# OpenwaterHealth/OpenLIFU-python

Hardware: AMD Instinct MI355X
Metric: Mvoxel-elements/s pressure-field accumulate (higher is better)
Workload: dtype f32-acc/f16x2+e4m3-corr

## Files before the change

### openlifu-python_amd/csrc/k_coset2.hip

```cpp
#include <algorithm>
#include <cstdlib>
#include "k_types.hip.h"
#include "olx_ctx.h"
#include "olx_launch.h"

namespace olx {

constexpr int CP_TW = 14;
constexpr int CP_TROWS = 26, CP_ROW0 = 15;
constexpr int CP_PSZ = 364;
constexpr int CP_UW = 12;
constexpr int CP_MT = 5;

#ifdef OLX_EXP_CUTRACE
static __device__ unsigned long long g_cutrace[16384][8][5];
#define OLX_CUTRACE(k, v) do { if (lane == 0 && blockIdx.y == 0 && blockIdx.x < 16384) g_cutrace[blockIdx.x][wave][k] = (v); } while (0)
#else
#define OLX_CUTRACE(k, v)
#endif

template <int MX, int MY, bool CLAMP, bool FP8, bool DIR = false, bool BOTH = true >
__global__ __launch_bounds__(COS_NW * 64, 4) void field_cosetp_k(
    const uint4* __restrict__ bfrag, float* __restrict__ pmag, float* __restrict__ inten,
    const int* __restrict__ targets ,
    const CosetBlock* __restrict__ blocks , const CosetParams P) {
    constexpr int NT = 2, THREADS = COS_NW * 64, PAIR = 2;
    constexpr int TROWS = CP_TROWS, ROW0 = CP_ROW0, PSZ = CP_PSZ, MT = CP_MT;
    static_assert((PSZ / 2) % 2 == 0 && ((PSZ / 2) % 32 == 22 || (PSZ / 2) % 32 == 30), "16 planes on 16 distinct even 8-byte slots");
    constexpr int RPR = 64 / CP_UW, NROUND = (TROWS + RPR - 1) / RPR;
    constexpr int B_KS_U4 = 128;
    constexpr int B_BYTES = PAIR * 4 * NT * B_KS_U4 * 16;
    constexpr int T_WORDS = COS_ZB * PSZ;
    __shared__ __attribute__((aligned(16))) unsigned char smem[B_BYTES + T_WORDS * 4 + T_WORDS * 4 + 64];
    auto s_B = [&](int rec, int nt, int part) -> const uint4* { return reinterpret_cast<const uint4*>(smem) + ((size_t)(rec * NT + nt) * B_KS_U4 + part * 64); };
    unsigned* const s_hi = reinterpret_cast<unsigned*>(smem + B_BYTES);
    unsigned* const s_lo = s_hi + T_WORDS;
    const int tile = blockIdx.y;
    const int tid = threadIdx.x, lane = tid & 63, wave = __builtin_amdgcn_readfirstlane(tid >> 6);
    const int g = lane >> 4, p16 = lane & 15;
    OLX_CUTRACE(2, __builtin_readcyclecounter());
    OLX_CUTRACE(0, (unsigned long long)__builtin_amdgcn_s_getreg((31 << 11) | 4));
    OLX_CUTRACE(1, (unsigned long long)__builtin_amdgcn_s_getreg((31 << 11) | 20));
    const int item = blockIdx.x;
    {
    const CosetBlock BK = blocks[item];
    const int npos = BK.npos, KY = BK.KY, ky_magic = BK.ky_magic;
    if (npos <= 0) return;
    const int ibase = BK.ibase, jbase = BK.jbase;
    const int k0 = BK.k0;
    const int ntile = __builtin_amdgcn_readfirstlane((npos - wave + COS_NW - 1) / COS_NW);
    const int lane_off = p16 * PSZ - g * CP_TW;
    int toff[MT];
#pragma unroll
    for (int t = 0; t < MT; ++t) {
        const int pos = min(wave + COS_NW * t, npos - 1);
        const int kx = (pos * ky_magic) >> 16, ky = pos - kx * KY;
        toff[t] = (ky + ROW0) * CP_TW + (CP_UW - 8 - 2 * kx);
    }
    floatx4_t acc[MT][NT];
#pragma unroll
    for (int t = 0; t < MT; ++t)
#pragma unroll
        for (int nt = 0; nt < NT; ++nt) acc[t][nt] = floatx4_t{0.f, 0.f, 0.f, 0.f};
    const int nsbp = P.nsbp;
    const int n_sb = P.nsa * nsbp;
    constexpr int CHUNK_U4 = PAIR * 4 * NT * B_KS_U4, PRE = CHUNK_U4 / THREADS;
    static_assert(CHUNK_U4 % THREADS == 0, "chunk must split evenly over the block");
    uint4 pre[PRE];
    const uint4* const bsrc = bfrag + (size_t)tile * n_sb * (4 * NT * B_KS_U4);
#pragma unroll
    for (int q = 0; q < PRE; ++q) {
        const int idx = tid + q * THREADS;
        pre[q] = idx < n_sb * 4 * NT * B_KS_U4 ? bsrc[idx] : make_uint4(0, 0, 0, 0);
    }
    OLX_STAMP(0);
    for (int sb0 = 0; sb0 < n_sb; sb0 += PAIR) {
        const int sa = sb0 / nsbp, sbb0 = sb0 - sa * nsbp;
        if (sb0 > 0) __syncthreads();
        if (sb0 == 0) OLX_STAMP(1);
        if (sb0 == 2) OLX_STAMP(7);
        if constexpr (FP8) __builtin_amdgcn_s_setprio(1);
        if (k0 + wave * COS_P < P.nz) {
            int lane_o = lane;
            asm volatile("" : "+v"(lane_o));
            const int wl = lane_o / CP_UW, ui = lane_o - CP_UW * wl;
            const bool gen_lane = wl < RPR;
            const int Ulane = ibase + P.x_begin + P.ux0 + P.mx * (ui - 7);
            const int Wlane = jbase + P.uy0 + P.my * (wl - ROW0);
            const int tw_off = (wave * COS_P) * PSZ + wl * CP_TW + (CP_UW - 1 - ui);
            float dz2[COS_P];
#pragma unroll
            for (int z = 0; z < COS_P; ++z) {
                const float dz = (float)(k0 + wave * COS_P + z) * P.hz - P.flat_ez;
                dz2[z] = dz * dz;
            }
            const float U = (float)(Ulane - 8 * P.mx * sa);
            const float dx = fmaf(U, P.hx_hi, fmaf(U, P.hx_lo, P.fx0));
            const float dx2 = dx * dx;
            const int Wsb = Wlane - 8 * P.my * sbb0;
            auto entry = [&](const float r2, const float dz2v, const float dy, const int o, const bool ok) __attribute__((always_inline)) {
                float d2 = r2 + dz2v;
                if (CLAMP) d2 = fmaxf(d2, P.dmin2);
                const float ri = __builtin_amdgcn_rsqf(d2);
                const float ph = d2 * ri;
                float rs = ri * P.g_scale;
                if constexpr (DIR) rs *= table_mod(dx, dy, ph, ri, P.dir_wx, P.dir_wy, P.absorb_l2);
                float gr = rs * __builtin_amdgcn_cosf(ph), gi = rs * __builtin_amdgcn_sinf(ph);
                asm volatile("" : "+v"(gr), "+v"(gi));
                half2_t hi;
                if constexpr (FP8) hi = __builtin_convertvector(float2_t{gr, gi}, half2_t);
                else hi = __builtin_bit_cast(half2_t, __builtin_amdgcn_cvt_pkrtz(gr, gi));
                float lr, li;
                const unsigned hw = __builtin_bit_cast(unsigned, hi);
                asm("v_fma_mix_f32 %0, %1, -1.0, %2 op_sel:[0,0,0] op_sel_hi:[1,0,0]" : "=v"(lr) : "v"(hw), "v"(gr));
                asm("v_fma_mix_f32 %0, %1, -1.0, %2 op_sel:[1,0,0] op_sel_hi:[1,0,0]" : "=v"(li) : "v"(hw), "v"(gi));
                unsigned lo_word;
                if constexpr (FP8) {
                    short2_t w;
                    w = __builtin_amdgcn_cvt_scalef32_pk_fp8_f32(w, lr, li, 1.0f / COS_F8_LO, false);
                    w = __builtin_amdgcn_cvt_scalef32_pk_fp8_f32(w, gr, gi, 1.0f / COS_F8_HI, true);
                    lo_word = __builtin_bit_cast(unsigned, w);
                } else {
                    lo_word = __builtin_bit_cast(unsigned, __builtin_amdgcn_cvt_pkrtz(lr, li));
                }
                if (ok && OLX_IN(o, T_WORDS, 0)) {
                    s_hi[o] = __builtin_bit_cast(unsigned, hi);
                    s_lo[o] = lo_word;
                }
            };
            static_assert((TROWS - 1) % RPR == 0 && COS_P <= RPR, "the last table row is shared by the planes of a wave");
#pragma unroll 2
            for (int r = 0; r < NROUND - 1; ++r) {
                const float W = (float)(Wsb + RPR * P.my * r);
                const float dy = fmaf(W, P.hy_hi, fmaf(W, P.hy_lo, P.fy0));
                const float r2 = fmaf(dy, dy, dx2);
#pragma unroll
                for (int z = 0; z < COS_P; ++z) entry(r2, dz2[z], dy, z * PSZ + tw_off + RPR * r * CP_TW, gen_lane);
            }
            if (KY + 14 >= TROWS - 1) {
                const float W = (float)(Wsb - P.my * wl + (TROWS - 1) * P.my);
                const float dy = fmaf(W, P.hy_hi, fmaf(W, P.hy_lo, P.fy0));
                float dzl = dz2[0];
#pragma unroll
                for (int z = 1; z < COS_P; ++z) dzl = wl == z ? dz2[z] : dzl;
                entry(fmaf(dy, dy, dx2), dzl, dy, (wave * COS_P + wl) * PSZ + (TROWS - 1) * CP_TW + (CP_UW - 1 - ui), wl < COS_P);
            }
        }
        if constexpr (FP8) __builtin_amdgcn_s_setprio(0);
#pragma unroll
        for (int q = 0; q < PRE; ++q) reinterpret_cast<uint4*>(smem)[tid + q * THREADS] = pre[q];
        if (sb0 == 0) OLX_STAMP(2);
        __syncthreads();
        if (sb0 == 0) OLX_STAMP(3);
        {
            const int nxt = (sb0 + PAIR) * 4 * NT * B_KS_U4, lim = n_sb * 4 * NT * B_KS_U4;
#pragma unroll
            for (int q = 0; q < PRE; ++q) {
                const int idx = nxt + tid + q * THREADS;
                if (idx < lim) pre[q] = bsrc[idx];
            }
        }
#pragma unroll
        for (int sl = 0; sl < PAIR; ++sl) {
            if (sbb0 + sl >= P.nsb) break;
            if constexpr (FP8) {
#pragma unroll
                for (int kb = 0; kb < 2; ++kb) {
                    Half8Bits bh[2][NT];
                    intx8_t b8[NT];
#pragma unroll
                    for (int nt = 0; nt < NT; ++nt) {
#pragma unroll
                        for (int ka = 0; ka < 2; ++ka) {
                            bh[ka][nt].u = s_B(sl * 4 + 2 * kb + ka, nt, 0)[lane];
                            const uint4 q = s_B(sl * 4 + 2 * kb + ka, nt, 1)[lane];
                            b8[nt][4 * ka + 0] = (int)q.x; b8[nt][4 * ka + 1] = (int)q.y; b8[nt][4 * ka + 2] = (int)q.z; b8[nt][4 * ka + 3] = (int)q.w;
                        }
                    }
// ... 44 lines not shown
                        if (t >= ntile) continue;
                        Half8Bits ah, al;
                        int lo_t = lane_off;
                        asm volatile("" : "+v"(lo_t));
                        const int ro = lo_t + toff[t];
                        if (!OLX_IN(ro + kso, T_WORDS - 3, 1)) continue;
                        const unsigned long long* ph2 = reinterpret_cast<const unsigned long long*>(s_hi + ro + kso);
                        const unsigned long long* pl2 = reinterpret_cast<const unsigned long long*>(s_lo + ro + kso);
                        const unsigned long long h0 = __hip_atomic_load(ph2, __ATOMIC_RELAXED, __HIP_MEMORY_SCOPE_WAVEFRONT);
                        const unsigned long long h1 = __hip_atomic_load(ph2 + 1, __ATOMIC_RELAXED, __HIP_MEMORY_SCOPE_WAVEFRONT);
                        const unsigned long long l0 = __hip_atomic_load(pl2, __ATOMIC_RELAXED, __HIP_MEMORY_SCOPE_WAVEFRONT);
                        const unsigned long long l1 = __hip_atomic_load(pl2 + 1, __ATOMIC_RELAXED, __HIP_MEMORY_SCOPE_WAVEFRONT);
                        ah.w[0] = (unsigned)h0; ah.w[1] = (unsigned)(h0 >> 32); ah.w[2] = (unsigned)h1; ah.w[3] = (unsigned)(h1 >> 32);
                        al.w[0] = (unsigned)l0; al.w[1] = (unsigned)(l0 >> 32); al.w[2] = (unsigned)l1; al.w[3] = (unsigned)(l1 >> 32);
#pragma unroll
                        for (int nt = 0; nt < NT; ++nt) acc[t][nt] = __builtin_amdgcn_mfma_f32_16x16x32_f16(ah.h, bh[nt].h, acc[t][nt], 0, 0, 0);
#pragma unroll
                        for (int nt = 0; nt < NT; ++nt) acc[t][nt] = __builtin_amdgcn_mfma_f32_16x16x32_f16(al.h, bh[nt].h, acc[t][nt], 0, 0, 0);
#pragma unroll
                        for (int nt = 0; nt < NT; ++nt) acc[t][nt] = __builtin_amdgcn_mfma_f32_16x16x32_f16(ah.h, bl[nt].h, acc[t][nt], 0, 0, 0);
                    }
                }
            }
        }
        if (sb0 == 0) OLX_STAMP(4);
    }
    OLX_STAMP(5);
    int lane_e = lane;
    asm volatile("" : "+v"(lane_e));
    const int c16 = lane_e >> 2;
    const int kz = k0 + 4 * (lane_e & 3);
    const int src_lane4 = (16 * (lane_e & 3) + (lane_e >> 2)) * 4;
    const float s_p = P.out_scale, s_i = P.out_scale * P.out_scale * P.inten_scale;
    const bool want_p = (P.flags & 1u) != 0, want_i = (P.flags & 2u) != 0;
#pragma unroll
    for (int t = 0; t < MT; ++t) {
        if (t >= ntile) continue;
        float o[NT][4];
#pragma unroll
        for (int r = 0; r < 4; r += 2) {
            const float2_t re = {acc[t][0][r], acc[t][0][r + 1]}, im = {acc[t][1][r], acc[t][1][r + 1]};
            const float2_t m = __builtin_elementwise_fma(re, re, im * im);
            o[0][r] = __builtin_amdgcn_sqrtf(m.x) * s_p;
            o[0][r + 1] = __builtin_amdgcn_sqrtf(m.y) * s_p;
            const float2_t in = m * float2_t{s_i, s_i};
            o[1][r] = in.x;
            o[1][r + 1] = in.y;
        }
#pragma unroll
        for (int nt = 0; nt < NT; ++nt) {
            floatx4_t v;
            v[0] = __builtin_bit_cast(float, __builtin_amdgcn_ds_bpermute(src_lane4, __builtin_bit_cast(int, o[nt][0])));
            v[1] = __builtin_bit_cast(float, __builtin_amdgcn_ds_bpermute(src_lane4, __builtin_bit_cast(int, o[nt][1])));
            v[2] = __builtin_bit_cast(float, __builtin_amdgcn_ds_bpermute(src_lane4, __builtin_bit_cast(int, o[nt][2])));
            v[3] = __builtin_bit_cast(float, __builtin_amdgcn_ds_bpermute(src_lane4, __builtin_bit_cast(int, o[nt][3])));
            acc[t][nt] = v;
        }
    }
    if (kz < P.nz) {
    const int4 tq = *reinterpret_cast<const int4*>(targets + ((size_t)tile * (MFMA_COLS * MFMA_MAX_NT) + c16) * 4);
    const int xm = P.nx - 1, ym = P.ny - 1;
    const int sxz = P.ny * P.nz;
    auto readout = [&](auto full_c) {
        constexpr bool FULL4 = decltype(full_c)::value != 0;
#pragma unroll
        for (int q = 0; q < 4; ++q) {
            const int code = q == 0 ? tq.x : q == 1 ? tq.y : q == 2 ? tq.z : tq.w;
            if (code < 0) continue;
            const unsigned m = (unsigned)code & 3u;
            const bool fx = (MX == 2) && (m & 1u), fy = (MY == 2) && ((MX == 2) ? (m >> 1) : (m & 1u));
            unsigned fxm = fx ? 0xFFFFFFFFu : 0u, fym = fy ? 0xFFFFFFFFu : 0u;
            asm volatile("" : "+v"(fxm), "+v"(fym));
            const long long fb = (long long)(code >> 2) * P.vox + kz;
            float* const base_p = pmag + fb;
            float* const base_i = inten + fb;
#pragma unroll
            for (int t = 0; t < MT; ++t) {
                if (t >= ntile) continue;
                const int pos = wave + COS_NW * t;
                const int kx = (pos * ky_magic) >> 16, ky = pos - kx * KY;
                const int i = ibase + 2 * P.mx * kx, j = jbase + P.my * ky;
                const unsigned o00 = (unsigned)(i * sxz + j * P.nz);
                const unsigned DX = (unsigned)((xm - 2 * i) * sxz), DY = (unsigned)((ym - 2 * j) * P.nz);
                const unsigned off = o00 + (fxm & DX) + (fym & DY);
                if (!OLX_IN(fb + off + (FULL4 ? 3 : 0), (long long)P.n_foci * P.vox, 2)) continue;
                if constexpr (FULL4) {
                    if (BOTH || want_p) *reinterpret_cast<floatx4u_t*>(base_p + off) = floatx4u_t{acc[t][0][0], acc[t][0][1], acc[t][0][2], acc[t][0][3]};
                    if (BOTH || want_i) *reinterpret_cast<floatx4u_t*>(base_i + off) = floatx4u_t{acc[t][1][0], acc[t][1][1], acc[t][1][2], acc[t][1][3]};
                } else {
#pragma unroll
                    for (int e = 0; e < 4; ++e)
                        if (kz + e < P.nz) {
                            if (BOTH || want_p) base_p[off + e] = acc[t][0][e];
                            if (BOTH || want_i) base_i[off + e] = acc[t][1][e];
                        }
                }
            }
        }
    };
    if (k0 + COS_ZB <= P.nz) readout(IntC<1>{}); else readout(IntC<0>{});
    }
    OLX_STAMP(6);
#ifdef OLX_EXP_CUTRACE
    OLX_CUTRACE(3, __builtin_readcyclecounter());
    asm volatile("s_waitcnt vmcnt(0)" ::: "memory");
    OLX_CUTRACE(4, __builtin_readcyclecounter());
#endif
    }
}

}

using namespace olx;
OLX_BOUNDS_READER(cosetp)

#ifdef OLX_EXP_CUTRACE
extern "C" int olx_exp_read_cutrace_cosetp(unsigned long long* out) {
    return (int)hipMemcpyFromSymbol(out, HIP_SYMBOL(olx::g_cutrace), sizeof(unsigned long long) * 16384 * 8 * 5);
}
#endif
#ifdef OLX_EXP_STAMPS
extern "C" int olx_exp_read_stamps_cosetp(unsigned long long* out) {
    return (int)hipMemcpyFromSymbol(out, HIP_SYMBOL(olx::g_stamps), sizeof(unsigned long long) * 4096 * 8);
}
#endif

template <int MX, int MY>
static void launch_cosetp(olx_ctx* c, const LatticePart& q, float* pm) {
    CosetParams Q = c->cp;
#ifdef OLX_DEBUG_BOUNDS
    if (getenv("OLX_DEBUG_BOUNDS_SELFTEST")) Q.n_foci -= 1;
#endif
    float* inten_exp = c->d_inten;
    const bool clamp = c->clamp || c->lat.clamp;
    dim3 grid(q.n_blocks, c->mp.n_tiles), blk(COS_NW * 64);
    const bool both = (Q.flags & 3u) == 3u;
#define OLX_CP(CL, F8, DR) do { if (both) hipLaunchKernelGGL((field_cosetp_k<MX, MY, CL, F8, DR, true>), grid, blk, 0, c->stream, q.bfrag, pm, inten_exp, c->d_targets, q.blocks, Q); \
                                else hipLaunchKernelGGL((field_cosetp_k<MX, MY, CL, F8, DR, false>), grid, blk, 0, c->stream, q.bfrag, pm, inten_exp, c->d_targets, q.blocks, Q); } while (0)
    if (c->dir_lattice) {
        if (clamp) OLX_CP(true, false, true); else OLX_CP(false, false, true);
    } else if (q.fp8) {
        if (clamp) OLX_CP(true, true, false); else OLX_CP(false, true, false);
    } else {
        if (clamp) OLX_CP(true, false, false); else OLX_CP(false, false, false);
    }
#undef OLX_CP
}

void olx_launch_cosetp(olx_ctx* c, const LatticePart& q, float* pm) {
    if (c->mx == 2 && c->my == 2) launch_cosetp<2, 2>(c, q, pm);
    else if (c->mx == 2) launch_cosetp<2, 1>(c, q, pm);
    else if (c->my == 2) launch_cosetp<1, 2>(c, q, pm);
    else launch_cosetp<1, 1>(c, q, pm);
}
```

### openlifu-python_amd/csrc/olx.hip

```cpp
#include "olx_ctx.h"

#include <dlfcn.h>
#include <unistd.h>

#include <algorithm>
#include <climits>
#include <cmath>
#include <cstring>
#include <thread>

#include "k_small.hip.h"
#include "olx_launch.h"
#include "olx_plan.h"
#include "k_toep.hip.h"

OLX_BOUNDS_READER(small)

template <class T> static int upload_if_changed(olx_ctx* c, DevBuf<T>& d, std::vector<T>& held, const std::vector<T>& v) {
    if (d.capacity() < v.size() || !d) held.clear();
    { int rc = d.reserve(c, v.size()); if (rc) return rc; }
    if (held.size() == v.size() && (v.empty() || !memcmp(held.data(), v.data(), sizeof(T) * v.size()))) return OLX_OK;
    HIPCHK(c, hipMemcpyAsync(d, v.data(), sizeof(T) * v.size(), hipMemcpyHostToDevice, c->stream));
    HIPCHK(c, hipStreamSynchronize(c->stream));
    held = v;
// ... 652 lines not shown
            L.ux0 = (int)std::llround(offx / c->grid.spacing[0]); L.uy0 = (int)std::llround(offy / c->grid.spacing[1]);
            L.fx0 = (float)((offx - L.ux0 * c->grid.spacing[0]) * rev); L.fy0 = (float)((offy - L.uy0 * c->grid.spacing[1]) * rev);
            const double hxw = c->grid.spacing[0] * rev, hyw = c->grid.spacing[1] * rev;
            L.hx_hi = (float)hxw; L.hx_lo = (float)(hxw - (double)L.hx_hi);
            L.hy_hi = (float)hyw; L.hy_lo = (float)(hyw - (double)L.hy_hi);
            L.hz = P.hz; L.dmin2 = P.dmin2; L.flat_ez = P.flat_ez;
            L.g_scale = M.g_scale; L.out_scale = M.out_scale; L.inten_scale = P.inten_scale;
            L.vox = P.vox; L.flags = P.flags;
            const long long tiles16 = coset_tiles16(P.nx - L.x_lo, P.ny - L.y_lo, A.mx, A.my, c->nt);
            c->fp8corr = fp8_want && c->use_coset && cos_fp8(c->nt) && !c->modifier();
            if (c->use_coset) {
                CosetParams& Q = c->cp;
                Q.nx = L.nx; Q.ny = L.ny; Q.nz = L.nz; Q.x_lo = L.x_lo; Q.y_lo = L.y_lo; Q.x_begin = L.x_begin; Q.mx = L.mx; Q.my = L.my;
                const int zb = COS_ZB;
                Q.xs = c->use_toep ? 1 : 2;
                olxplan::ToepPlan tp{};
                c->toep_nm = 1;
                int kyw = COS_KYW;
                if (c->use_toep) {
                    int saw_pin = 0, nm_pin = 0;
#ifdef OLX_DEV_PINS
                    if (const char* e = getenv("OLX_EXP_TOEP_SAW")) { const int v = atoi(e); if (v >= 8 && v <= 24) saw_pin = v; }
                    if (const char* e = getenv("OLX_EXP_TOEP_NM")) nm_pin = atoi(e) == 3 ? 3 : 1;
#endif
                    tp = olxplan::toep_plan(A.ax, Q.mx, Q.my, Q.xs, Q.nx - Q.x_lo, Q.ny - Q.y_lo, Q.nz, c->dir_lattice, saw_pin, nm_pin);
                    c->toep_nm = tp.nm; kyw = tp.kyw;
                }
                const int kxw = c->use_toep ? 8 * c->toep_nm : cos_kxw(c->nt);
                olxplan::coset_partition(Q, kxw, zb, kyw);
                Q.nsa = L.nsa; Q.nsb = L.nsb; Q.nsbp = L.nsbp; Q.ux0 = L.ux0; Q.uy0 = L.uy0; Q.fx0 = L.fx0; Q.fy0 = L.fy0;
                Q.hx_hi = L.hx_hi; Q.hx_lo = L.hx_lo; Q.hy_hi = L.hy_hi; Q.hy_lo = L.hy_lo; Q.hz = L.hz;
                Q.dmin2 = L.dmin2; Q.flat_ez = L.flat_ez; Q.g_scale = L.g_scale; Q.out_scale = L.out_scale; Q.inten_scale = L.inten_scale;
                Q.vox = L.vox; Q.flags = L.flags; Q.n_foci = F;
                Q.dir_wx = (c->dir_lattice && c->directivity) ? (float)(0.5 * c->h_size[0] / lambda) : 0.f;
                Q.dir_wy = (c->dir_lattice && c->directivity) ? (float)(0.5 * c->h_size[1] / lambda) : 0.f;
                Q.absorb_l2 = c->dir_lattice ? (float)(c->absorb_np_m * lambda * 1.4426950408889634) : 0.f;
                {
                    const std::vector<int> jobs = olxplan::build_store_jobs(tiles, MFMA_MAX_NT, MFMA_COLS, COS_JOBS, (P.flags & OLX_OUT_PMAG) != 0, (P.flags & OLX_OUT_INTENSITY) != 0);
                    int rc = upload_if_changed(c, c->d_jobs, c->up_jobs, jobs);
                    if (rc) return rc;
                }
                {
                    auto pick_grp = [&](int kblocks) {
                        const unsigned long long nb = (unsigned long long)Q.xs * Q.mx * Q.my * Q.nsx * Q.nsy * kblocks;
                        for (int g2 = std::min(kblocks, 32); g2 >= 2; --g2) if (kblocks % g2 == 0 && nb % (8ull * g2) == 0) return (unsigned)g2;
                        return 1u;
                    };
                    const int kcut = c->fp8corr ? c->fp8_kcut : 0;
                    const int kb_near = kcut / zb, kb_far = Q.kblocks - kb_near;
                    unsigned kgrp = pick_grp(kb_far), kgrp_near = kb_near > 0 ? pick_grp(kb_near) : 0u;
#ifdef OLX_DEV_PINS
                    if (const char* e = getenv("OLX_EXP_KGRP")) { kgrp = (unsigned)std::max(1, atoi(e)); if (kb_near > 0) kgrp_near = kgrp; }
#endif
                    const int rec_key[16] = {Q.nx, Q.ny, Q.nz, Q.x_lo, Q.y_lo, Q.mx, Q.my, Q.nsx, Q.nsy, Q.kblocks, zb, (int)kgrp, c->use_cosetp ? 40 : 0, Q.xs, kcut, (int)kgrp_near};
                    std::vector<CosetBlock> blk;
                    if (!c->up_blocks.empty() && memcmp(c->up_blocks_key, rec_key, sizeof rec_key) == 0) blk = c->up_blocks;
                    else {
                        std::string why;
                        CosetParams Qf = Q; Qf.kblocks = kb_far;
                        if (!olxplan::build_coset_blocks(Qf, zb, kgrp, c->use_cosetp ? 40 : 0, blk, why))
                            return fail(c, OLX_ESTATE, "kernel 2g: %s", why.c_str());
                        for (CosetBlock& b : blk) b.k0 += kcut;
                        if (kb_near > 0) {
                            std::vector<CosetBlock> near;
                            CosetParams Qn = Q; Qn.kblocks = kb_near;
                            if (!olxplan::build_coset_blocks(Qn, zb, kgrp_near, c->use_cosetp ? 40 : 0, near, why))
// ... 18 lines not shown
                    c->toep_ksmask = tp.ks_mask;
                    const int ksteps_total = tp.ksteps_total, e4_units = tp.e4_units;
                    for (int q = 0; q < 4; ++q) c->toep_targets[q] = tiles[0][0].tgt[q];
                    { int rc = c->d_cell.reserve(c, A.cell.size()); if (rc) return rc; }
                    HIPCHK(c, hipMemcpy(c->d_cell, A.cell.data(), sizeof(int) * A.cell.size(), hipMemcpyHostToDevice));
                    c->afrag_half = (size_t)ntiles * c->toep_nsa * 8 * A.nsb * 4 * 64;
                    { int rc = c->d_afrag.reserve(c, 2 * c->afrag_half); if (rc) return rc; }
                    long long n_mfma = 0;
                    const int wx = P.nx - L.x_lo, wy = P.ny - L.y_lo;
                    const double units_e4m3 = c->toep_nm == 2 ? 3.0 : (double)ksteps_total + (double)e4_units;
                    const double per_row = far_frac * units_e4m3 + (1.0 - far_frac) * 3.0 * ksteps_total;
                    for (int rx = 0; rx < Q.xs * A.mx; ++rx)
                        for (int ry = 0; ry < A.my; ++ry) {
                            const int kxa = rx < wx ? (wx - 1 - rx) / (Q.xs * A.mx) + 1 : 0, kya = ry < wy ? (wy - 1 - ry) / A.my + 1 : 0;
                            for (int sx = 0; sx < Q.nsx; ++sx)
                                for (int sy = 0; sy < Q.nsy; ++sy) {
                                    const int KX = (sx + 1) * kxa / Q.nsx - sx * kxa / Q.nsx, KY = (sy + 1) * kya / Q.nsy - sy * kya / Q.nsy;
                                    if (KX > 0 && KY > 0) n_mfma += (long long)((double)KY * per_row * (c->toep_nm > 1 ? 8 * c->toep_nm : 8) * A.nsb * Q.kblocks);
                                }
                        }
                    snprintf(nmbuf, sizeof nmbuf, "field_toep%s_k<mx%d,my%d,flat,%s%s> %d columns for %d foci x %d images in %d tile(s); "
                             "%dx%d lattice, pitch %dx%d voxels, %lld MFMA/launch (%lld dense), %d row tile(s) x %d y positions per block", "", c->mx, c->my, lat_clamp ? "clamp" : "noclamp", f8tag.c_str(),
                             total_cols, F, n_img, ntiles, A.ax, A.ay, A.mx, A.my, n_mfma, n_dense, c->toep_nm, kyw);
                } else {
                long long n_mfma = (long long)((double)tiles16 * ((P.nz + COS_P - 1) / COS_P) * A.nsa * A.nsb * 4 * c->nt * corr_units * ntiles);
                if (c->use_cosetp) {
                    long long npos_all = 0;
                    const int wx = P.nx - L.x_lo, wy = P.ny - L.y_lo;
                    for (int rx = 0; rx < 2 * A.mx; ++rx)
                        for (int ry = 0; ry < A.my; ++ry)
                            npos_all += (long long)(rx < wx ? (wx - 1 - rx) / (2 * A.mx) + 1 : 0) * (ry < wy ? (wy - 1 - ry) / A.my + 1 : 0);
                    n_mfma = (long long)((double)npos_all * Q.kblocks * A.nsa * A.nsb * 4 * c->nt * corr_units * ntiles);
                }
                snprintf(nmbuf, sizeof nmbuf, "field_coset%s_k<nt%d,mx%d,my%d,flat,%s%s%s> %d columns for %d foci x %d images in %d tile(s); "
                         "%dx%d lattice, pitch %dx%d voxels, %lld MFMA/launch (%lld dense)", c->use_cosetp ? "p" : "", c->nt, c->mx, c->my, lat_clamp ? "clamp" : "noclamp",
                         f8tag.c_str(), "", total_cols, F, n_img, ntiles, A.ax, A.ay, A.mx, A.my, n_mfma, n_dense);
                }
            } else {
                const long long n_mfma = (long long)L.tiles_x * L.tiles_y * L.kgroups * A.nsa * A.nsb * 4 * c->lat_mt * c->nt * 3 * ntiles;
                snprintf(nmbuf, sizeof nmbuf, "field_lattice_k<mt%d,nt%d,mx%d,my%d,flat,%s> %d columns for %d foci x %d images in %d tile(s); "
                         "%dx%d lattice, pitch %dx%d voxels, %lld MFMA/launch", c->lat_mt, c->nt, c->mx, c->my, lat_clamp ? "clamp" : "noclamp",
                         total_cols, F, n_img, ntiles, A.ax, A.ay, A.mx, A.my, n_mfma);
            }
        } else {
            snprintf(nmbuf, sizeof nmbuf, "field_mfma_k<mt%d,nt%d,mx%d,my%d,%s,%s> %d columns for %d foci x %d images in %d tile(s)",
                     P.nz >= 48 ? 4 : 1, c->nt, c->mx, c->my, c->flat ? "flat" : "general", c->clamp ? "clamp" : (c->near ? "near" : "noclamp"), total_cols, F,
                     n_img, ntiles);
        }
    } else if (c->mx * c->my * c->nf == 1) {
        if (c->modifier()) snprintf(nmbuf, sizeof nmbuf, "field_accum_dir_k<4,%s> (%s%s%s)", c->clamp ? "clamp" : "noclamp", c->directivity ? "piston directivity" : "",
                                    (c->directivity && c->absorb_np_m > 0) ? ", " : "", c->absorb_np_m > 0 ? "uniform absorption" : "");
        else snprintf(nmbuf, sizeof nmbuf, "field_accum_k<4,%s,%s>", c->flat ? "flat" : "general", c->clamp ? "clamp" : (c->near ? "near" : "noclamp"));
    } else {
        const std::vector<int> perm = olxplan::mirror_perms(n, nm, c->dx == 2, c->dy == 2, c->h_px.data(), c->h_py.data(), nm);
        int rc = upload_if_changed(c, c->d_perm, c->up_perm, perm);
        if (!rc) rc = c->d_tab.reserve(c, (size_t)((F + c->nf - 1) / c->nf) * n * (SH_HEAD + 2 * nm * c->nf));
        if (rc) return rc;
        snprintf(nmbuf, sizeof nmbuf, "field_shared_k<4,mx%d,my%d,dx%d,dy%d,nf%d,%s,%s>", c->mx, c->my, c->dx, c->dy, c->nf,
                 c->flat ? "flat" : "general", c->clamp ? "clamp" : (c->near ? "near" : "noclamp"));
    }
    if (c->modifier() && c->use_mfma && !(c->use_lattice && c->use_coset)) {
        c->dir_lattice = false; c->allow_shared = false;
        return configure_variant_impl(c);
    }
    if (c->directivity && c->use_mfma) strncat(nmbuf, " +piston directivity in the tables", sizeof nmbuf - strlen(nmbuf) - 1);
    if (c->absorb_np_m > 0 && c->use_mfma) strncat(nmbuf, " +uniform absorption in the tables", sizeof nmbuf - strlen(nmbuf) - 1);
    c->variant = nmbuf;
    return OLX_OK;
}
// ... 111 lines not shown
    char nm[128];
    snprintf(nm, sizeof nm, "field_pulse_k (pulsed: %d samples, %.4g samples per burst)", c->pulse_nt, P.tdt);
    c->variant = nm;
    c->packed_version = ~0ull;
    c->planned = true; c->uploaded = false;
    return OLX_OK;
}

extern "C" {

int olx_field_plan(olx_ctx* c, const olx_grid* g, const olx_slab* slab, int n_foci, double freq, double cs,
                   double rho, double p0_pa, unsigned flags) {
    if (!c) return OLX_EINVAL;
    if (c->n_el <= 0) return fail(c, OLX_ESTATE, "olx_field_plan: call olx_set_elements first");
    if (c->n_foci <= 0) return fail(c, OLX_ESTATE, "olx_field_plan: no steering table (olx_bf_solve / olx_set_steering)");
    if (!g) return fail(c, OLX_EINVAL, "olx_field_plan: null grid");
    if (n_foci != c->n_foci) return fail(c, OLX_EINVAL, "olx_field_plan: n_foci %d != steering table foci %d", n_foci, c->n_foci);
    for (int a = 0; a < 3; ++a)
        if (g->n[a] < 1 || !(g->spacing[a] > 0)) return fail(c, OLX_EINVAL, "olx_field_plan: bad grid axis %d", a);
    if (!(freq > 0) || !(cs > 0) || !(rho > 0)) return fail(c, OLX_EINVAL, "olx_field_plan: freq, c, rho must be > 0");
    if (!(flags & (OLX_OUT_PMAG | OLX_OUT_INTENSITY | OLX_OUT_COMPLEX))) return fail(c, OLX_EINVAL, "olx_field_plan: no outputs selected");
    if (c->pulse_nt > 0) return plan_pulse(c, g, slab, n_foci, freq, cs, rho, p0_pa, flags);
    if (flags & OLX_OUT_PMAX) return fail(c, OLX_EINVAL, "olx_field_plan: OLX_OUT_PMAX needs a pulsed plan (olx_field_pulse)");
    if (flags & OLX_OUT_PII) return fail(c, OLX_EINVAL, "olx_field_plan: OLX_OUT_PII needs a pulsed plan (olx_field_pulse)");
    if (flags & ~(OLX_OUT_PMAG | OLX_OUT_INTENSITY | OLX_OUT_COMPLEX | OLX_FIELD_FP8_CORRECTION | OLX_FIELD_FP16_CORRECTION | OLX_FIELD_DIRECTIVITY)) return fail(c, OLX_EINVAL, "olx_field_plan: unknown flag bits 0x%x", flags);
    if ((flags & OLX_FIELD_DIRECTIVITY) && c->h_xaxis.size() != 3 * (size_t)c->n_el)
        return fail(c, OLX_ESTATE, "olx_field_plan: OLX_FIELD_DIRECTIVITY needs olx_set_element_apertures");
    olx_slab s{0, g->n[0]};
    if (slab) s = *slab;
    if (s.x_begin < 0 || s.x_count < 1 || s.x_begin + s.x_count > g->n[0]) return fail(c, OLX_EINVAL, "olx_field_plan: slab outside grid");
    HIPCHK(c, hipSetDevice(c->device));
    {
        std::string env;
        for (const char* name : {"OLX_FIELD_VARIANT", "OLX_FP8_CORRECTION", "OLX_EXP_TOEP_SAW", "OLX_EXP_TOEP_NM", "OLX_EXP_KGRP", "OLX_INTENSITY_STORED"}) { const char* e = getenv(name); env += e ? e : ""; env += '|'; }
        const bool same = c->planned && !c->uploaded && !c->hetero && !c->pulsed && memcmp(&c->grid, g, sizeof *g) == 0 && c->slab.x_begin == s.x_begin &&
                          c->slab.x_count == s.x_count && c->plan_foci == n_foci && c->freq == freq && c->c == cs && c->rho == rho &&
                          c->p0_pa == p0_pa && c->flags == flags && c->plan_absorb == c->absorb_np_m && c->nbuf == (c->comm_active() ? olx_ctx::NBUF : 1) && c->plan_env == env;
        c->plan_env = env;
        if (same) {
            c->agg_local = -1; c->agg_total = 0;
            if (c->packed_version != c->steer_version) return configure_variant(c);
            return OLX_OK;
        }
    }
    HIPCHK(c, hipStreamSynchronize(c->stream));
    c->grid = *g; c->slab = s; c->plan_foci = n_foci; c->hetero = false;
    c->pulsed = false; c->pmax_live = false; c->agg_pmax_valid = false; c->pii_live = false;
    c->agg_local = -1; c->agg_total = 0;
    c->freq = freq; c->c = cs; c->rho = rho; c->p0_pa = p0_pa; c->flags = flags; c->plan_absorb = c->absorb_np_m;
    const long long vox = (long long)s.x_count * g->n[1] * g->n[2];
    pii_regrid(c, vox);
    const size_t total = (size_t)vox * n_foci;
    c->nbuf = c->comm_active() ? olx_ctx::NBUF : 1;
    { const char* pin = getenv("OLX_INTENSITY_STORED"); c->derive_i = (flags & OLX_OUT_INTENSITY) && !(pin && *pin && strcmp(pin, "0") != 0); }
    c->inten_live = false;
    { int rc = reserve_outputs(c, total, c->nbuf, (flags & OLX_OUT_INTENSITY) && !c->derive_i, (flags & OLX_OUT_COMPLEX) != 0, true); if (rc) return rc; }
    if (c->derive_i) c->d_inten.release();
    { int rc = c->d_tab.reserve(c, (size_t)n_foci * c->n_el * TAB_STRIDE); if (rc) return rc; }
    FieldParams& P = c->fp;
    P.nx = s.x_count; P.ny = g->n[1]; P.nz = g->n[2]; P.n_el = c->n_el;
    P.x_begin = s.x_begin;
    const double rev = freq / cs;
    P.hx = (float)(g->spacing[0] * rev); P.hy = (float)(g->spacing[1] * rev); P.hz = (float)(g->spacing[2] * rev);
    const double dmin = 0.5 * std::min({g->spacing[0], g->spacing[1], g->spacing[2]});
    P.dmin2 = (float)(dmin * dmin * rev * rev);
    P.inten_scale = (float)(1e-4 / (2.0 * rho * cs));
    P.vox = vox; P.flags = ((flags & 7u) | OLX_OUT_PMAG) & ~(c->derive_i ? (unsigned)OLX_OUT_INTENSITY : 0u);
// ... 2012 lines not shown
```

### openlifu-python_amd/csrc/olx_params.h

```cpp
#pragma once
#ifdef __HIPCC__
#include <hip/hip_runtime.h>
#endif
#include <stdint.h>

namespace olx {

constexpr int BF_THREADS = 256;
constexpr int SH_HEAD = 8;
constexpr int TAB_STRIDE = 8;
constexpr int FIELD_THREADS = 256;

struct FieldParams {
    int nx, ny, nz;
    int n_el;
    int x_begin;
    float hx, hy, hz;
    float dmin2;
    float inten_scale;
    float flat_ez;
    float flat_kz, flat_fz;
    float absorb_l2;
    long long vox;
    unsigned flags;
// ... 34 lines not shown
    int kgroups;
    int nsa, nsb;
    int nsbp;
    int ux0, uy0;
    float fx0, fy0;
    float hx_hi, hx_lo, hy_hi, hy_lo, hz;
    float dmin2, flat_ez, g_scale, out_scale, inten_scale;
    long long vox;
    unsigned flags;
};

constexpr int LAT_ELEMS_LDS = 128;
constexpr int LAT_TW = 10;
constexpr int LAT_PSZ = 116;
constexpr int LAT_THREADS = 512;

struct CosetParams {
    int nx, ny, nz;
    int x_lo, y_lo, x_begin;
    int mx, my;
    int nsx, nsy;
    int xs;
    int kblocks;
    int nsa, nsb;
    int nsbp;
    int ux0, uy0;
    float fx0, fy0, hx_hi, hx_lo, hy_hi, hy_lo, hz;
    float dmin2, flat_ez, g_scale, out_scale, inten_scale;
    float dir_wx, dir_wy;
    float absorb_l2;
    long long vox;
    unsigned flags;
    int n_foci;
};

struct CosetBlock {
    int ibase, jbase;
    int k0;
    int npos;
    int KY;
    int ky_magic;
    int KX;
    int pad_;
};

constexpr int COS_NW = 8;
constexpr int COS_P = 2;
constexpr int COS_ZB = COS_NW * COS_P;
constexpr int COS_KYW = 11;
constexpr int COS_JOBS = 64;
constexpr int cos_kxw(int nt) { return nt >= 4 ? 2 : (nt >= 2 ? 3 : 6); }
constexpr bool cos_fp8(int nt) { return nt <= 2; }
constexpr float COS_F8_LO = 32.0f, COS_F8_HI = 1.0f / 64.0f;

constexpr int HET_TAB_HEAD = 12;

struct HeteroParams {
    int n_planes;
    int n_layers;
    int n_foci;
    float u0, v0;
    float inv_hx, inv_hy;
    int nxg, nyg;
    int xg_begin;
    float kappa;
};
// ... 76 lines not shown
```

Before: 109.8 million.

## Reuse overlapping Green's-table columns across sub-blocks and add pressure-only kernel variant

When the sub-block pair count equals two, each later sub-block shifts the overlapping four columns of the per-plane Green's table in LDS instead of recomputing them. Only the eight new columns are evaluated, which cuts the transcendental and conversion work per fill. The lane-to-entry mapping is reworked to cover the tail rows. A separate PONLY template variant drops the intensity computation and stores when only pressure is requested. The change adds LDS moves plus a wavefront fence, and depends on the reuse geometry being correct.

```diff
diff --git a/openlifu-python_amd/csrc/k_coset2.hip b/openlifu-python_amd/csrc/k_coset2.hip
--- a/openlifu-python_amd/csrc/k_coset2.hip
+++ b/openlifu-python_amd/csrc/k_coset2.hip
@@ -10,6 +10,7 @@
 constexpr int CP_TROWS = 26, CP_ROW0 = 15;
 constexpr int CP_PSZ = 364;
 constexpr int CP_UW = 12;
+constexpr int CP_SHARED = 4;
 constexpr int CP_MT = 5;
 
 #ifdef OLX_EXP_CUTRACE
@@ -19,15 +20,16 @@
 #define OLX_CUTRACE(k, v)
 #endif
 
-template <int MX, int MY, bool CLAMP, bool FP8, bool DIR = false, bool BOTH = true >
+template <int MX, int MY, bool CLAMP, bool FP8, bool DIR = false, bool BOTH = true ,
+          bool PONLY = false >
 __global__ __launch_bounds__(COS_NW * 64, 4) void field_cosetp_k(
     const uint4* __restrict__ bfrag, float* __restrict__ pmag, float* __restrict__ inten,
     const int* __restrict__ targets ,
     const CosetBlock* __restrict__ blocks , const CosetParams P) {
     constexpr int NT = 2, THREADS = COS_NW * 64, PAIR = 2;
+    static_assert(!(BOTH && PONLY), "one output or both");
     constexpr int TROWS = CP_TROWS, ROW0 = CP_ROW0, PSZ = CP_PSZ, MT = CP_MT;
     static_assert((PSZ / 2) % 2 == 0 && ((PSZ / 2) % 32 == 22 || (PSZ / 2) % 32 == 30), "16 planes on 16 distinct even 8-byte slots");
-    constexpr int RPR = 64 / CP_UW, NROUND = (TROWS + RPR - 1) / RPR;
     constexpr int B_KS_U4 = 128;
     constexpr int B_BYTES = PAIR * 4 * NT * B_KS_U4 * 16;
     constexpr int T_WORDS = COS_ZB * PSZ;
@@ -64,6 +66,10 @@
         for (int nt = 0; nt < NT; ++nt) acc[t][nt] = floatx4_t{0.f, 0.f, 0.f, 0.f};
     const int nsbp = P.nsbp;
     const int n_sb = P.nsa * nsbp;
+    bool reuse_ok = nsbp == PAIR;
+#ifdef OLX_DEV_PINS
+    reuse_ok = reuse_ok && P.cp_noreuse == 0;
+#endif
     constexpr int CHUNK_U4 = PAIR * 4 * NT * B_KS_U4, PRE = CHUNK_U4 / THREADS;
     static_assert(CHUNK_U4 % THREADS == 0, "chunk must split evenly over the block");
     uint4 pre[PRE];
@@ -77,28 +83,20 @@
     for (int sb0 = 0; sb0 < n_sb; sb0 += PAIR) {
         const int sa = sb0 / nsbp, sbb0 = sb0 - sa * nsbp;
         if (sb0 > 0) __syncthreads();
+        const bool reuse = sb0 > 0 && reuse_ok;
         if (sb0 == 0) OLX_STAMP(1);
         if (sb0 == 2) OLX_STAMP(7);
         if constexpr (FP8) __builtin_amdgcn_s_setprio(1);
         if (k0 + wave * COS_P < P.nz) {
             int lane_o = lane;
             asm volatile("" : "+v"(lane_o));
-            const int wl = lane_o / CP_UW, ui = lane_o - CP_UW * wl;
-            const bool gen_lane = wl < RPR;
-            const int Ulane = ibase + P.x_begin + P.ux0 + P.mx * (ui - 7);
-            const int Wlane = jbase + P.uy0 + P.my * (wl - ROW0);
-            const int tw_off = (wave * COS_P) * PSZ + wl * CP_TW + (CP_UW - 1 - ui);
             float dz2[COS_P];
 #pragma unroll
             for (int z = 0; z < COS_P; ++z) {
                 const float dz = (float)(k0 + wave * COS_P + z) * P.hz - P.flat_ez;
                 dz2[z] = dz * dz;
             }
-            const float U = (float)(Ulane - 8 * P.mx * sa);
-            const float dx = fmaf(U, P.hx_hi, fmaf(U, P.hx_lo, P.fx0));
-            const float dx2 = dx * dx;
-            const int Wsb = Wlane - 8 * P.my * sbb0;
-            auto entry = [&](const float r2, const float dz2v, const float dy, const int o, const bool ok) __attribute__((always_inline)) {
+            auto entry = [&](const float r2, const float dz2v, const float dx, const float dy, const int o, const bool ok) __attribute__((always_inline)) {
                 float d2 = r2 + dz2v;
                 if (CLAMP) d2 = fmaxf(d2, P.dmin2);
                 const float ri = __builtin_amdgcn_rsqf(d2);
@@ -128,22 +126,66 @@
                     s_lo[o] = lo_word;
                 }
             };
-            static_assert((TROWS - 1) % RPR == 0 && COS_P <= RPR, "the last table row is shared by the planes of a wave");
+            auto fill = [&](auto reuse_c) __attribute__((always_inline)) {
+                constexpr bool RU = decltype(reuse_c)::value != 0;
+                constexpr int CW = RU ? CP_UW - CP_SHARED : CP_UW;
+                constexpr int RPF = 64 / CW;
+                constexpr int NRF = (TROWS - (RU ? COS_P : 1)) / RPF;
+                static_assert(NRF * RPF == TROWS - (RU ? COS_P : 1) && (RU ? COS_P * COS_P : COS_P) <= RPF, "the tail rows fit one evaluation of the wave's planes");
+                const int wl = lane_o / CW, ui = lane_o - CW * wl;
+                const bool gen_lane = wl < RPF;
+                const int Ulane = ibase + P.x_begin + P.ux0 + P.mx * (ui - 7);
+                const int Wlane = jbase + P.uy0 + P.my * (wl - ROW0);
+                const int tw_off = (wave * COS_P) * PSZ + wl * CP_TW + (CP_UW - 1 - ui);
+                const float U = (float)(Ulane - 8 * P.mx * sa);
+                const float dx = fmaf(U, P.hx_hi, fmaf(U, P.hx_lo, P.fx0));
+                const float dx2 = dx * dx;
+                const int Wsb = Wlane - 8 * P.my * sbb0;
 #pragma unroll 2
-            for (int r = 0; r < NROUND - 1; ++r) {
-                const float W = (float)(Wsb + RPR * P.my * r);
-                const float dy = fmaf(W, P.hy_hi, fmaf(W, P.hy_lo, P.fy0));
-                const float r2 = fmaf(dy, dy, dx2);
-#pragma unroll
-                for (int z = 0; z < COS_P; ++z) entry(r2, dz2[z], dy, z * PSZ + tw_off + RPR * r * CP_TW, gen_lane);
-            }
-            if (KY + 14 >= TROWS - 1) {
-                const float W = (float)(Wsb - P.my * wl + (TROWS - 1) * P.my);
-                const float dy = fmaf(W, P.hy_hi, fmaf(W, P.hy_lo, P.fy0));
-                float dzl = dz2[0];
-#pragma unroll
-                for (int z = 1; z < COS_P; ++z) dzl = wl == z ? dz2[z] : dzl;
-                entry(fmaf(dy, dy, dx2), dzl, dy, (wave * COS_P + wl) * PSZ + (TROWS - 1) * CP_TW + (CP_UW - 1 - ui), wl < COS_P);
+                for (int r = 0; r < NRF; ++r) {
+                    const float W = (float)(Wsb + RPF * P.my * r);
+                    const float dy = fmaf(W, P.hy_hi, fmaf(W, P.hy_lo, P.fy0));
+                    const float r2 = fmaf(dy, dy, dx2);
+#pragma unroll
+                    for (int z = 0; z < COS_P; ++z) entry(r2, dz2[z], dx, dy, z * PSZ + tw_off + RPF * r * CP_TW, gen_lane);
+                }
+                const bool last_row = KY + 14 >= TROWS - 1;
+                if constexpr (RU) {
+                    const int zt = wl >> 1, rowt = TROWS - COS_P + (wl & 1);
+                    const float W = (float)(Wsb - P.my * wl + rowt * P.my);
+                    const float dy = fmaf(W, P.hy_hi, fmaf(W, P.hy_lo, P.fy0));
+                    float dzl = dz2[0];
+#pragma unroll
+                    for (int z = 1; z < COS_P; ++z) dzl = zt == z ? dz2[z] : dzl;
+                    entry(fmaf(dy, dy, dx2), dzl, dx, dy, (wave * COS_P + zt) * PSZ + rowt * CP_TW + (CP_UW - 1 - ui), zt < COS_P && (last_row || rowt < TROWS - 1));
+                } else if (last_row) {
+                    const float W = (float)(Wsb - P.my * wl + (TROWS - 1) * P.my);
+                    const float dy = fmaf(W, P.hy_hi, fmaf(W, P.hy_lo, P.fy0));
+                    float dzl = dz2[0];
+#pragma unroll
+                    for (int z = 1; z < COS_P; ++z) dzl = wl == z ? dz2[z] : dzl;
+                    entry(fmaf(dy, dy, dx2), dzl, dx, dy, (wave * COS_P + wl) * PSZ + (TROWS - 1) * CP_TW + (CP_UW - 1 - ui), wl < COS_P);
+                }
+            };
+            if (reuse) {
+                static_assert(COS_P * TROWS <= 64 && CP_UW - CP_SHARED == 8 && CP_TW % 2 == 0 && PSZ % 2 == 0, "one lane per (plane, row); aligned 8-byte moves");
+                const int zm = lane_o >= TROWS ? 1 : 0;
+                const int mo = (wave * COS_P + zm) * PSZ + (lane_o - zm * TROWS) * CP_TW;
+                if (lane_o < COS_P * TROWS && OLX_IN(mo, T_WORDS - (CP_UW - 1), 3)) {
+                    unsigned long long mv[4];
+                    __builtin_memcpy(&mv[0], __builtin_assume_aligned(s_hi + mo + 8, 8), 8);
+                    __builtin_memcpy(&mv[1], __builtin_assume_aligned(s_hi + mo + 10, 8), 8);
+                    __builtin_memcpy(&mv[2], __builtin_assume_aligned(s_lo + mo + 8, 8), 8);
+                    __builtin_memcpy(&mv[3], __builtin_assume_aligned(s_lo + mo + 10, 8), 8);
+                    __builtin_memcpy(__builtin_assume_aligned(s_hi + mo, 8), &mv[0], 8);
+                    __builtin_memcpy(__builtin_assume_aligned(s_hi + mo + 2, 8), &mv[1], 8);
+                    __builtin_memcpy(__builtin_assume_aligned(s_lo + mo, 8), &mv[2], 8);
+                    __builtin_memcpy(__builtin_assume_aligned(s_lo + mo + 2, 8), &mv[3], 8);
+                }
+                __builtin_amdgcn_fence(__ATOMIC_RELEASE, "wavefront");
+                fill(IntC<1>{});
+            } else {
+                fill(IntC<0>{});
             }
         }
         if constexpr (FP8) __builtin_amdgcn_s_setprio(0);
@@ -254,23 +296,26 @@
     const int kz = k0 + 4 * (lane_e & 3);
     const int src_lane4 = (16 * (lane_e & 3) + (lane_e >> 2)) * 4;
     const float s_p = P.out_scale, s_i = P.out_scale * P.out_scale * P.inten_scale;
-    const bool want_p = (P.flags & 1u) != 0, want_i = (P.flags & 2u) != 0;
+    const bool want_p = PONLY || (P.flags & 1u) != 0, want_i = !PONLY && (P.flags & 2u) != 0;
+    constexpr int NOUT = PONLY ? 1 : NT;
 #pragma unroll
     for (int t = 0; t < MT; ++t) {
         if (t >= ntile) continue;
-        float o[NT][4];
+        float o[NOUT][4];
 #pragma unroll
         for (int r = 0; r < 4; r += 2) {
             const float2_t re = {acc[t][0][r], acc[t][0][r + 1]}, im = {acc[t][1][r], acc[t][1][r + 1]};
             const float2_t m = __builtin_elementwise_fma(re, re, im * im);
             o[0][r] = __builtin_amdgcn_sqrtf(m.x) * s_p;
             o[0][r + 1] = __builtin_amdgcn_sqrtf(m.y) * s_p;
-            const float2_t in = m * float2_t{s_i, s_i};
-            o[1][r] = in.x;
-            o[1][r + 1] = in.y;
-        }
-#pragma unroll
-        for (int nt = 0; nt < NT; ++nt) {
+            if constexpr (!PONLY) {
+                const float2_t in = m * float2_t{s_i, s_i};
+                o[1][r] = in.x;
+                o[1][r + 1] = in.y;
+            }
+        }
+#pragma unroll
+        for (int nt = 0; nt < NOUT; ++nt) {
             floatx4_t v;
             v[0] = __builtin_bit_cast(float, __builtin_amdgcn_ds_bpermute(src_lane4, __builtin_bit_cast(int, o[nt][0])));
             v[1] = __builtin_bit_cast(float, __builtin_amdgcn_ds_bpermute(src_lane4, __builtin_bit_cast(int, o[nt][1])));
@@ -307,14 +352,14 @@
                 const unsigned off = o00 + (fxm & DX) + (fym & DY);
                 if (!OLX_IN(fb + off + (FULL4 ? 3 : 0), (long long)P.n_foci * P.vox, 2)) continue;
                 if constexpr (FULL4) {
-                    if (BOTH || want_p) *reinterpret_cast<floatx4u_t*>(base_p + off) = floatx4u_t{acc[t][0][0], acc[t][0][1], acc[t][0][2], acc[t][0][3]};
-                    if (BOTH || want_i) *reinterpret_cast<floatx4u_t*>(base_i + off) = floatx4u_t{acc[t][1][0], acc[t][1][1], acc[t][1][2], acc[t][1][3]};
+                    if (BOTH || PONLY || want_p) *reinterpret_cast<floatx4u_t*>(base_p + off) = floatx4u_t{acc[t][0][0], acc[t][0][1], acc[t][0][2], acc[t][0][3]};
+                    if (!PONLY && (BOTH || want_i)) *reinterpret_cast<floatx4u_t*>(base_i + off) = floatx4u_t{acc[t][1][0], acc[t][1][1], acc[t][1][2], acc[t][1][3]};
                 } else {
 #pragma unroll
                     for (int e = 0; e < 4; ++e)
                         if (kz + e < P.nz) {
-                            if (BOTH || want_p) base_p[off + e] = acc[t][0][e];
-                            if (BOTH || want_i) base_i[off + e] = acc[t][1][e];
+                            if (BOTH || PONLY || want_p) base_p[off + e] = acc[t][0][e];
+                            if (!PONLY && (BOTH || want_i)) base_i[off + e] = acc[t][1][e];
                         }
                 }
             }
@@ -356,9 +401,10 @@
     float* inten_exp = c->d_inten;
     const bool clamp = c->clamp || c->lat.clamp;
     dim3 grid(q.n_blocks, c->mp.n_tiles), blk(COS_NW * 64);
-    const bool both = (Q.flags & 3u) == 3u;
-#define OLX_CP(CL, F8, DR) do { if (both) hipLaunchKernelGGL((field_cosetp_k<MX, MY, CL, F8, DR, true>), grid, blk, 0, c->stream, q.bfrag, pm, inten_exp, c->d_targets, q.blocks, Q); \
-                                else hipLaunchKernelGGL((field_cosetp_k<MX, MY, CL, F8, DR, false>), grid, blk, 0, c->stream, q.bfrag, pm, inten_exp, c->d_targets, q.blocks, Q); } while (0)
+    const bool both = (Q.flags & 3u) == 3u, ponly = (Q.flags & 3u) == 1u;
+#define OLX_CP(CL, F8, DR) do { if (both) hipLaunchKernelGGL((field_cosetp_k<MX, MY, CL, F8, DR, true, false>), grid, blk, 0, c->stream, q.bfrag, pm, inten_exp, c->d_targets, q.blocks, Q); \
+                                else if (ponly) hipLaunchKernelGGL((field_cosetp_k<MX, MY, CL, F8, DR, false, true>), grid, blk, 0, c->stream, q.bfrag, pm, inten_exp, c->d_targets, q.blocks, Q); \
+                                else hipLaunchKernelGGL((field_cosetp_k<MX, MY, CL, F8, DR, false, false>), grid, blk, 0, c->stream, q.bfrag, pm, inten_exp, c->d_targets, q.blocks, Q); } while (0)
     if (c->dir_lattice) {
         if (clamp) OLX_CP(true, false, true); else OLX_CP(false, false, true);
     } else if (q.fp8) {
diff --git a/openlifu-python_amd/csrc/olx.hip b/openlifu-python_amd/csrc/olx.hip
--- a/openlifu-python_amd/csrc/olx.hip
+++ b/openlifu-python_amd/csrc/olx.hip
@@ -708,6 +708,9 @@
                 Q.hx_hi = L.hx_hi; Q.hx_lo = L.hx_lo; Q.hy_hi = L.hy_hi; Q.hy_lo = L.hy_lo; Q.hz = L.hz;
                 Q.dmin2 = L.dmin2; Q.flat_ez = L.flat_ez; Q.g_scale = L.g_scale; Q.out_scale = L.out_scale; Q.inten_scale = L.inten_scale;
                 Q.vox = L.vox; Q.flags = L.flags; Q.n_foci = F;
+#ifdef OLX_DEV_PINS
+                { const char* e = getenv("OLX_EXP_CP_NOREUSE"); Q.cp_noreuse = (e && atoi(e) != 0) ? 1 : 0; }
+#endif
                 Q.dir_wx = (c->dir_lattice && c->directivity) ? (float)(0.5 * c->h_size[0] / lambda) : 0.f;
                 Q.dir_wy = (c->dir_lattice && c->directivity) ? (float)(0.5 * c->h_size[1] / lambda) : 0.f;
                 Q.absorb_l2 = c->dir_lattice ? (float)(c->absorb_np_m * lambda * 1.4426950408889634) : 0.f;
@@ -792,9 +795,14 @@
                             npos_all += (long long)(rx < wx ? (wx - 1 - rx) / (2 * A.mx) + 1 : 0) * (ry < wy ? (wy - 1 - ry) / A.my + 1 : 0);
                     n_mfma = (long long)((double)npos_all * Q.kblocks * A.nsa * A.nsb * 4 * c->nt * corr_units * ntiles);
                 }
+#ifdef OLX_DEV_PINS
+                const char* const noreuse_tag = (c->use_cosetp && Q.cp_noreuse) ? ",noreuse" : "";
+#else
+                const char* const noreuse_tag = "";
+#endif
                 snprintf(nmbuf, sizeof nmbuf, "field_coset%s_k<nt%d,mx%d,my%d,flat,%s%s%s> %d columns for %d foci x %d images in %d tile(s); "
                          "%dx%d lattice, pitch %dx%d voxels, %lld MFMA/launch (%lld dense)", c->use_cosetp ? "p" : "", c->nt, c->mx, c->my, lat_clamp ? "clamp" : "noclamp",
-                         f8tag.c_str(), "", total_cols, F, n_img, ntiles, A.ax, A.ay, A.mx, A.my, n_mfma, n_dense);
+                         f8tag.c_str(), noreuse_tag, total_cols, F, n_img, ntiles, A.ax, A.ay, A.mx, A.my, n_mfma, n_dense);
                 }
             } else {
                 const long long n_mfma = (long long)L.tiles_x * L.tiles_y * L.kgroups * A.nsa * A.nsb * 4 * c->lat_mt * c->nt * 3 * ntiles;
@@ -972,7 +980,7 @@
     HIPCHK(c, hipSetDevice(c->device));
     {
         std::string env;
-        for (const char* name : {"OLX_FIELD_VARIANT", "OLX_FP8_CORRECTION", "OLX_EXP_TOEP_SAW", "OLX_EXP_TOEP_NM", "OLX_EXP_KGRP", "OLX_INTENSITY_STORED"}) { const char* e = getenv(name); env += e ? e : ""; env += '|'; }
+        for (const char* name : {"OLX_FIELD_VARIANT", "OLX_FP8_CORRECTION", "OLX_EXP_TOEP_SAW", "OLX_EXP_TOEP_NM", "OLX_EXP_KGRP", "OLX_INTENSITY_STORED", "OLX_EXP_CP_NOREUSE"}) { const char* e = getenv(name); env += e ? e : ""; env += '|'; }
         const bool same = c->planned && !c->uploaded && !c->hetero && !c->pulsed && memcmp(&c->grid, g, sizeof *g) == 0 && c->slab.x_begin == s.x_begin &&
                           c->slab.x_count == s.x_count && c->plan_foci == n_foci && c->freq == freq && c->c == cs && c->rho == rho &&
                           c->p0_pa == p0_pa && c->flags == flags && c->plan_absorb == c->absorb_np_m && c->nbuf == (c->comm_active() ? olx_ctx::NBUF : 1) && c->plan_env == env;
diff --git a/openlifu-python_amd/csrc/olx_params.h b/openlifu-python_amd/csrc/olx_params.h
--- a/openlifu-python_amd/csrc/olx_params.h
+++ b/openlifu-python_amd/csrc/olx_params.h
@@ -90,6 +90,9 @@
     long long vox;
     unsigned flags;
     int n_foci;
+#ifdef OLX_DEV_PINS
+    int cp_noreuse;
+#endif
 };
 
 struct CosetBlock {
```

After: 113.6 million (median of 6 runs). 1.04x the previous value.
